# Sukikui/PTI-LDM-VAE

Measured on AMD Instinct MI355X. Metric: vae_train_images_per_sec_256x256, higher is better.
Workload: dtype fp16 forward operands + activations / bf16 backward operands + gradients, fp32 accumulate; 1 GPU; config/vae_dente_no_adv.json 256x256x1 batch 32/GPU: fwd + L1 + 1e-3*KL + bwd + all-reduce + Adam (perceptual term omitted: --perceptual times it; adversarial branch inactive before epoch 6, --adv times it); global_batch=32, parallelism=dp1

## Files before the change

### pti_ldm_vae_amd/csrc/wgrad_mfma.hip

```cpp
#include "pti_common.h"

namespace {

constexpr int TH = 8, TW = 16;
constexpr int PTI_WGRAD_SLAB_V4 = 1 << 30;
#ifndef PTI_WGRAD_BATCH_MAX
#define PTI_WGRAD_BATCH_MAX 16
#endif

struct WgArgs {
  const bf16* x;
  const bf16* dy;
  const stat_t* in_stats;
  const float* gamma;
  const float* beta;
  float* slab;
  int N, H, W, Cin, Ho, Wo, Cout;
  int mode, prologue, groups;
  float eps, inv_cnt;
  int tiles_x, tiles_y, ntiles, S;
  int ci_tiles;
  long long slab_stride;
  int x_f16;
  int diag;
// ... 983 lines not shown
  const int jb = gword & 15, split = gword >> 4, cc = pos - b.grp_start[xcd][gi];
  const W4Job& a = b.job[jb];
  const int ci_pairs = a.Cin / (32 * C::NCH);
  typedef short v4s __attribute__((ext_vector_type(4)));
  typedef short v8s __attribute__((ext_vector_type(8)));
  __shared__ __attribute__((aligned(16))) unsigned char smem[C::LDS];
  const unsigned lds0 = (unsigned)(size_t)(__attribute__((address_space(3))) unsigned char*)smem;
  const int tid = threadIdx.x, lane = tid & 63;
  const int w8 = __builtin_amdgcn_readfirstlane(tid >> 6);
  const int cb = w8 % C::NCB, ch = (w8 / C::NCB) % C::NCH, rg = w8 / (C::NCB * C::NCH);
  const int cotb = cc / ci_pairs, citb = cc % ci_pairs;
  const int co0 = cotb * 32 * C::NCB, ci0 = citb * 32 * C::NCH;
  const bool do_bias = (citb == 0) && (ch == 0);

  int H = a.H, W = a.W;
  asm volatile("" : "+s"(H), "+s"(W));
  int ldsoff[C::NSLOT];
  int yy[C::NSLOT], xx[C::NSLOT], rel[C::NSLOT];
  bool pv[C::NSLOT];
  {
    const int pix = lane >> 2, piece = lane & 3;
#pragma unroll
    for (int k = 0; k < C::KX; ++k) {
      const int xi = w8 + 8 * k;
      const bool sink = xi >= C::NX;
      const int h = xi / C::XI, i = xi - C::XI * h, p = 16 * i + pix;
      ldsoff[k] = sink ? C::STG : h * C::XSUB + i * 1024;
      pv[k] = !sink && p < C::NPX;
      yy[k] = p / HWp - 1;
      xx[k] = p - (p / HWp) * HWp - 1;
      rel[k] = (yy[k] * W + xx[k]) * a.Cin * 2 + (ci0 + h * 32 + piece * 8) * 2;
    }
#pragma unroll
    for (int k = C::KX; k < C::NSLOT; ++k) {
      const int di = w8 + 8 * (k - C::KX), c = di / C::TH_, i = di % C::TH_;
      ldsoff[k] = C::XB + c * C::DSUB + i * 1024;
      pv[k] = true;
      yy[k] = i;
      xx[k] = pix;
      rel[k] = (i * W + pix) * a.Cout * 2 + (co0 + c * 32 + piece * 8) * 2;
    }
#pragma unroll
    for (int k = 0; k < C::NSLOT; ++k) ldsoff[k] = __builtin_amdgcn_readfirstlane(ldsoff[k]);
  }
  const unsigned char* xb = reinterpret_cast<const unsigned char*>(a.x);
  const unsigned char* db = reinterpret_cast<const unsigned char*>(a.dy);
  const unsigned char* zero = reinterpret_cast<const unsigned char*>(pti_wgrad_zero_page);
  struct TilePos { const unsigned char* xt; const unsigned char* dt; int oy0, ox0; };
  auto locate = [&](int tile) -> TilePos {
    TilePos tp;
    const bool live = tile < a.ntiles;
    int t = live ? tile : 0;
    const int tx_ = t % a.tiles_x; t /= a.tiles_x;
    const int ty_ = t % a.tiles_y;
    const int n = t / a.tiles_y;
    tp.oy0 = live ? ty_ * C::TH_ : 1 << 24; tp.ox0 = tx_ * TW;
    const size_t pix0 = (size_t)(n * H + ty_ * C::TH_) * W + tp.ox0;
    tp.xt = xb + pix0 * a.Cin * 2;
    tp.dt = db + pix0 * a.Cout * 2;
    return tp;
  };
  auto issue_slot = [&](const TilePos& tp, int stage, int k) {
    if (b.diag & 1) return;
    const unsigned sb = __builtin_amdgcn_readfirstlane(lds0 + stage * C::STGS + ldsoff[k]);
    const bool ok = pv[k] && (unsigned)(tp.oy0 + yy[k]) < (unsigned)H && (unsigned)(tp.ox0 + xx[k]) < (unsigned)W;
    glds16(ok ? (k < C::KX ? tp.xt : tp.dt) + rel[k] : zero, sb);
  };

  f32x16 acc[3][3];
  float bsum = 0.f;
#pragma unroll
  for (int r = 0; r < 16; ++r)
#pragma unroll
    for (int kh = 0; kh < 3; ++kh)
#pragma unroll
      for (int kw = 0; kw < 3; ++kw) acc[kh][kw][r] = 0.f;
  const int g = lane >> 4, q = (lane & 15) >> 2, pp = lane & 3;
  const int fbase = (8 * (g >> 1) + q) * PP + (16 * (g & 1) + 4 * pp) * 2;
  auto tr_frag = [&](const unsigned char* p) -> bf16x8 {
    const v4s d0 = __builtin_amdgcn_ds_read_tr16_b64_v4i16((v4s __attribute__((address_space(3)))*)(p));
    const v4s d1 = __builtin_amdgcn_ds_read_tr16_b64_v4i16((v4s __attribute__((address_space(3)))*)(p + 4 * PP));
    const v8s t = {d0[0], d0[1], d0[2], d0[3], d1[0], d1[1], d1[2], d1[3]};
    return __builtin_bit_cast(bf16x8, t);
  };

  const int ntl = a.ntiles > split ? (a.ntiles - split + a.S - 1) / a.S : 0;
  auto tile_of = [&](int k) { return k < ntl ? split + k * a.S : a.ntiles; };
#pragma unroll
  for (int s = 0; s < C::DP; ++s) {
    const TilePos tp = locate(tile_of(s));
#pragma unroll
    for (int k = 0; k < C::NSLOT; ++k) issue_slot(tp, s, k);
  }
  bf16x8 dfr[4], xcur, xq1;
  auto xfrag_at = [&](const unsigned char* lX, int f) { return tr_frag(lX + fbase + ((4 * rg + f / 3) * HWp + f % 3) * PP); };
  auto dfrag_at = [&](const unsigned char* lS, int r) { return tr_frag(lS + C::XB + cb * C::DSUB + fbase + (4 * rg + r) * TW * PP); };
  wait_vmcnt<C::NSLOT * (C::DP - 1)>();
  __builtin_amdgcn_s_barrier();
#pragma unroll
  for (int r = 0; r < 4; ++r) dfr[r] = dfrag_at(smem, r);
  xcur = xfrag_at(smem + ch * C::XSUB, 0);
  xq1 = xfrag_at(smem + ch * C::XSUB, 1);

  int ps = 0;
  for (int it = 0; it < ntl; ++it) {
    int fs = ps + C::DP;
    fs = fs >= C::NST ? fs - C::NST : fs;
    const int ns = ps + 1 == C::NST ? 0 : ps + 1;
    const TilePos ft = locate(tile_of(it + C::DP));
    wait_vmcnt<C::NSLOT * (C::DP - 2)>();
    __builtin_amdgcn_s_barrier();
    const unsigned char* lX = smem + ps * C::STGS + ch * C::XSUB;
    const unsigned char* lN = smem + ns * C::STGS;
    if (b.diag & 2) {
#pragma unroll
      for (int k = 0; k < C::NSLOT; ++k) issue_slot(ft, fs, k);
      ps = ns;
      continue;
    }
    if (do_bias) {
#pragma unroll
      for (int r = 0; r < 4; ++r) {
        const u32x4 dwv = __builtin_bit_cast(u32x4, dfr[r]);
        float s8 = 0.f;
#pragma unroll
        for (int i = 0; i < 4; ++i) s8 += __uint_as_float(dwv[i] << 16) + __uint_as_float(dwv[i] & 0xffff0000u);
        bsum += s8;
      }
    }
    bf16x8 dnx[4];
#pragma unroll
    for (int f = 0; f < 18; ++f) {
      const int rr = f / 3, kw = f % 3;
      bf16x8 xq2 = f + 2 < 18 ? xfrag_at(lX, f + 2) : xfrag_at(lN + ch * C::XSUB, f + 2 - 18);
      if (kw == 0 && rr >= 2) dnx[rr - 2] = dfrag_at(lN, rr - 2);
#pragma unroll
      for (int kh = 0; kh < 3; ++kh) {
        const int r = rr - kh;
        if (r >= 0 && r < 4) acc[kh][kw] = __builtin_amdgcn_mfma_f32_32x32x16_bf16(dfr[r], xcur, acc[kh][kw], 0, 0, 0);
      }
      if (C::NSLOT == 4) {
        if (f == 2) issue_slot(ft, fs, 0);
        if (f == 6) issue_slot(ft, fs, 1);
        if (f == 10) issue_slot(ft, fs, 2);
        if (f == 14) issue_slot(ft, fs, 3);
      } else {
        if (f == 2) issue_slot(ft, fs, 0);
        if (f == 5) issue_slot(ft, fs, 1);
        if (f == 8) issue_slot(ft, fs, 2);
        if (f == 11) issue_slot(ft, fs, 3);
        if (f == 14) issue_slot(ft, fs, C::NSLOT - 1);
      }
      if (kw == 0 && rr >= 2) __builtin_amdgcn_sched_group_barrier(0x100, 4, 0);
      else __builtin_amdgcn_sched_group_barrier(0x100, 2, 0);
      {
        const int nm = (rr == 0 || rr == 5) ? 1 : ((rr == 1 || rr == 4) ? 2 : 3);
        if (nm == 3) __builtin_amdgcn_sched_group_barrier(0x008, 3, 0);
        else if (nm == 2) __builtin_amdgcn_sched_group_barrier(0x008, 2, 0);
        else __builtin_amdgcn_sched_group_barrier(0x008, 1, 0);
      }
      __builtin_amdgcn_sched_barrier(0);
      xcur = xq1;
      xq1 = xq2;
    }
#pragma unroll
    for (int r = 0; r < 4; ++r) dfr[r] = dnx[r];
    ps = ns;
  }
  wait_vmcnt<0>();

  const int ci = lane & 31, hsel = lane >> 5;
  if (do_bias) bsum += __shfl_xor(bsum, 32, 64);
  if constexpr (C::NRG == 2) {
    __syncthreads();
    float* red = reinterpret_cast<float*>(smem) + (cb + C::NCB * ch) * 5120;
    float* bred = reinterpret_cast<float*>(smem) + C::NCB * C::NCH * 5120;
#pragma unroll
    for (int round = 0; round < 2; ++round) {
      if (round) __syncthreads();
      if (rg == 1) {
#pragma unroll
        for (int t = 0; t < 9; ++t)
          if ((t < 5) == (round == 0))
#pragma unroll
            for (int q4 = 0; q4 < 4; ++q4)
              *(f32x4*)(red + (t - 5 * round) * 1024 + ci * 32 + (((2 * q4 + hsel) ^ (ci & 7)) << 2)) =
                  f32x4{acc[t / 3][t % 3][4 * q4], acc[t / 3][t % 3][4 * q4 + 1], acc[t / 3][t % 3][4 * q4 + 2], acc[t / 3][t % 3][4 * q4 + 3]};
        if (round == 0 && do_bias && lane < 32) bred[cb * 32 + lane] = bsum;
      }
      __syncthreads();
      if (rg == 0) {
#pragma unroll
        for (int t = 0; t < 9; ++t)
          if ((t < 5) == (round == 0))
#pragma unroll
            for (int q4 = 0; q4 < 4; ++q4) {
              const f32x4 v = *(const f32x4*)(red + (t - 5 * round) * 1024 + ci * 32 + (((2 * q4 + hsel) ^ (ci & 7)) << 2));
#pragma unroll
              for (int j = 0; j < 4; ++j) acc[t / 3][t % 3][4 * q4 + j] += v[j];
            }
        if (round == 0 && do_bias && lane < 32) bsum += bred[cb * 32 + lane];
      }
    }
    if (rg == 1) return;
  }
  const int cc32 = (C::NCB * cotb + cb) * (a.Cin / 32) + C::NCH * citb + ch;
  float* blk = a.slab + (size_t)split * a.slab_stride + (size_t)cc32 * 9216;
#pragma unroll
  for (int kh = 0; kh < 3; ++kh)
#pragma unroll
    for (int kw = 0; kw < 3; ++kw)
#pragma unroll
      for (int q4 = 0; q4 < 4; ++q4)
        *(f32x4*)(blk + (kh * 3 + kw) * 1024 + ci * 32 + (((2 * q4 + hsel) ^ (ci & 7)) << 2)) =
            f32x4{acc[kh][kw][4 * q4], acc[kh][kw][4 * q4 + 1], acc[kh][kw][4 * q4 + 2], acc[kh][kw][4 * q4 + 3]};
  if (do_bias && lane < 32) a.slab[(size_t)split * a.slab_stride + (size_t)9 * a.Cout * a.Cin + co0 + cb * 32 + lane] = bsum;
}

__global__ __launch_bounds__(256) void wgrad_reduce4_kernel(W4Batch b) {
  __shared__ f32x4 red[16][16];
  int jb = 0;
  while (jb + 1 < b.njobs && (int)blockIdx.x >= b.first_rblk[jb + 1]) ++jb;
  const W4Job& a = b.job[jb];
  const float* __restrict__ slab = a.slab;
  float* __restrict__ dw = b.dw[jb];
  float* __restrict__ dbias = b.dbias[jb];
  const int S = a.S, Cout = a.Cout, Cin = a.Cin, accumulate = b.accumulate[jb];
  const long long stride = a.slab_stride;
  const long long total = (long long)9 * Cout * Cin;
  const int col = threadIdx.x & 15, sg = threadIdx.x >> 4;
  const long long e = ((long long)(blockIdx.x - b.first_rblk[jb]) * 16 + col) * 4;
  f32x4 s0 = {0.f, 0.f, 0.f, 0.f}, s1 = s0;
  if (e < total + Cout) {
    int k = sg;
    for (; k + 16 < S; k += 32) {
      s0 += *(const f32x4*)(slab + (size_t)k * stride + e);
      s1 += *(const f32x4*)(slab + (size_t)(k + 16) * stride + e);
    }
    if (k < S) s0 += *(const f32x4*)(slab + (size_t)k * stride + e);
  }
  red[sg][col] = s0 + s1;
  __syncthreads();
  if (sg == 0 && e < total + Cout) {
    f32x4 sum = red[0][col];
#pragma unroll
    for (int g = 1; g < 16; ++g) sum += red[g][col];
    if (e < total) {
      const int cc = (int)(e / 9216), i = (int)(e % 9216);
      const int ci_tiles = Cin / 32;
      const int co0 = (cc / ci_tiles) * 32, ci0 = (cc % ci_tiles) * 32;
      const int tap = i >> 10, ci = (i >> 5) & 31, cog = ((i >> 2) & 7) ^ (ci & 7);
#pragma unroll
      for (int j = 0; j < 4; ++j) {
        const size_t o = ((size_t)(co0 + cog * 4 + j) * Cin + ci0 + ci) * 9 + tap;
        dw[o] = accumulate ? dw[o] + sum[j] : sum[j];
      }
    } else if (dbias) {
      const int co = (int)(e - total);
#pragma unroll
      for (int j = 0; j < 4; ++j) dbias[co + j] = accumulate ? dbias[co + j] + sum[j] : sum[j];
    }
  }
}

__global__ __launch_bounds__(256) void wgrad_reduce_kernel(const float* __restrict__ slab, long long stride, int S,
                                                           float* __restrict__ dw, float* __restrict__ dbias, int Cout,
                                                           int Cin, int KK, int accumulate) {
  __shared__ f32x4 red[16][16];
  const long long total = (long long)KK * Cout * Cin;
  const int col = threadIdx.x & 15, sg = threadIdx.x >> 4;
  const long long e = ((long long)blockIdx.x * 16 + col) * 4;
  f32x4 s0 = {0.f, 0.f, 0.f, 0.f}, s1 = s0;
  if (e < total + Cout) {
    int k = sg;
    for (; k + 16 < S; k += 32) {
      s0 += *(const f32x4*)(slab + (size_t)k * stride + e);
      s1 += *(const f32x4*)(slab + (size_t)(k + 16) * stride + e);
    }
    if (k < S) s0 += *(const f32x4*)(slab + (size_t)k * stride + e);
  }
  red[sg][col] = s0 + s1;
  __syncthreads();
  if (sg == 0 && e < total + Cout) {
    f32x4 sum = red[0][col];
#pragma unroll
    for (int g = 1; g < 16; ++g) sum += red[g][col];
    if (e < total) {
      const int ci = e % Cin;
      const int co = (e / Cin) % Cout;
      const int t = e / ((long long)Cin * Cout);
#pragma unroll
      for (int j = 0; j < 4; ++j) {
        const size_t o = ((size_t)co * Cin + ci + j) * KK + t;
        dw[o] = accumulate ? dw[o] + sum[j] : sum[j];
      }
    } else if (dbias) {
      const int co = (int)(e - total);
#pragma unroll
      for (int j = 0; j < 4; ++j) dbias[co + j] = accumulate ? dbias[co + j] + sum[j] : sum[j];
    }
  }
}

template <int KS, int S_, int CO_T, int CI_T>
void launch_w(const WgArgs& a, int grid_y, hipStream_t st) {
  if (a.prologue == PTI_PRO_NONE)
    PTI_LAUNCH((wgrad_mfma_kernel<KS, S_, CO_T, CI_T, true>), dim3(grid_y, a.S), dim3(256), 0, st, a);
  else
    PTI_LAUNCH((wgrad_mfma_kernel<KS, S_, CO_T, CI_T, false>), dim3(grid_y, a.S), dim3(256), 0, st, a);
}
template <int KS, int S_>
void launch_wt(const WgArgs& a, int co_t, int ci_t, int grid_y, hipStream_t st) {
  if (co_t == 64 && ci_t == 64) launch_w<KS, S_, 64, 64>(a, grid_y, st);
  else if (co_t == 64) launch_w<KS, S_, 64, 32>(a, grid_y, st);
  else if (ci_t == 64) launch_w<KS, S_, 32, 64>(a, grid_y, st);
  else launch_w<KS, S_, 32, 32>(a, grid_y, st);
}

}

static int w6_mode(int n, int h, int w, int cin, int cout) {
  const char* e = getenv("PTI_WGRAD_V6");
  const int v = e ? atoi(e) : 3;
  if (v >= 1 && cout % 128 == 0 && cin % 64 == 0) return 2;
  if (v >= 2 && cout % 64 == 0 && cin % 64 == 0 && (v == 2 || (long long)h * w <= 128 * 128)) return 3;
  return 0;
}
static void w4_fill_job(W4Job& a, const void* x, const void* dy, int n, int h, int w, int cin, int cout, int mode) {
  a.x = (const bf16*)x; a.dy = (const bf16*)dy; a.slab = nullptr;
  a.N = n; a.H = h; a.W = w; a.Cin = cin; a.Cout = cout;
  a.tiles_x = cdiv(w, TW); a.tiles_y = cdiv(h, mode == 2 ? W6A::TH_ : TH); a.ntiles = n * a.tiles_x * a.tiles_y;
  a.slab_stride = (long long)9 * cout * cin + cout;
  a.S = 1;
  a.cob2 = mode;
}
static bool w4_eligible(int n, int h, int w, int cin, int cout) {
  return n > 0 && h > 0 && w > 0 && cin > 0 && cout > 0 && cin % 32 == 0 && cout % 32 == 0 &&
         (long long)n * h * w * cin * 2 < (1ll << 31) && (long long)n * h * w * cout * 2 < (1ll << 31);
}
static int w4_mode(int cout) {
  static const int cob2_env = getenv("PTI_WGRAD_V4_COB2") ? atoi(getenv("PTI_WGRAD_V4_COB2")) : 1;
  return (cob2_env && cout % 64 == 0) ? 1 : 0;
}
extern "C" int pti_conv_wgrad_batched_mode(int n, int h, int w, int cin, int cout) {
  if (!w4_eligible(n, h, w, cin, cout)) return PTI_EUNSUPPORTED;
  const int v4 = w4_mode(cout), v6 = w6_mode(n, h, w, cin, cout);
  return v6 ? v6 : v4;
}
static int wgrad_diag_env() {
  const char* v = getenv("PTI_WGRAD_V4_DIAG");
  const char* ok = getenv("PTI_ALLOW_WRONG_RESULTS");
  if (!v || atoi(v) == 0) return 0;
  if (!ok || atoi(ok) != 1) {
    fprintf(stderr, "[pti] PTI_WGRAD_V4_DIAG ignored: it needs PTI_ALLOW_WRONG_RESULTS=1 (results are garbage)\n");
    return 0;
  }
  fprintf(stderr, "[pti] WRONG-RESULT DIAGNOSTIC ACTIVE: PTI_WGRAD_V4_DIAG=%s\n", v);
  return atoi(v);
}
static long long w4_plan(W4Batch& b, float* workspace, long long workspace_floats) {
  static const int wgs_env = getenv("PTI_WGRAD_V4_WGS") ? atoi(getenv("PTI_WGRAD_V4_WGS")) : 2048;
  static const int diag_env = wgrad_diag_env();
  b.diag = diag_env;
  auto tiles32 = [](const W4Job& a) {
    return a.cob2 == 2 ? (a.Cin / 64) * (a.Cout / 128) : a.cob2 == 3 ? (a.Cin / 64) * (a.Cout / 64)
                                                                     : (a.Cin / 32) * (a.Cout / (a.cob2 ? 64 : 32));
  };
  const bool m6 = b.njobs > 0 && b.job[0].cob2 >= 2;
  const char* w6e = getenv("PTI_WGRAD_V6_WGS");
  const int wgs6 = w6e && atoi(w6e) > 0 ? atoi(w6e) : 512;
  double work = 0;
  for (int j = 0; j < b.njobs; ++j) work += (double)tiles32(b.job[j]) * (b.job[j].cob2 == 1 ? 2 : 1) * b.job[j].ntiles;
  double per_wg = work / wgs_env > 2.0 ? work / wgs_env : 2.0;
  if (m6) per_wg = work / wgs6 > 4.0 ? work / wgs6 : 4.0;
  for (int attempt = 0;; ++attempt) {
    long long used = 0;
    int rb = 0, groups = 0;
    bool fits = true;
    for (int j = 0; j < b.njobs; ++j) {
      W4Job& a = b.job[j];
      int S = (int)((double)a.ntiles * (a.cob2 == 1 ? 2 : 1) / per_wg + 0.5);
      if (S > a.ntiles / (a.cob2 ? 1 : 2)) S = a.ntiles / (a.cob2 ? 1 : 2);
      if (S > 255) S = 255;
      if (S < 1) S = 1;
      if (used + (long long)S * a.slab_stride > workspace_floats) fits = false;
      a.S = S;
      a.slab = workspace + used;
      used += (long long)S * a.slab_stride;
      groups += S;
      b.first_rblk[j] = rb;
      rb += (int)((a.slab_stride / 4 + 15) / 16);
    }
    b.first_rblk[b.njobs] = rb;
    if (fits && groups <= 8 * W4_MAXGRP) {
      int len[8] = {0, 0, 0, 0, 0, 0, 0, 0};
      for (int x = 0; x < 8; ++x) { b.ngrp[x] = 0; b.grp_start[x][0] = 0; }
      int order[PTI_WGRAD_BATCH_MAX];
      for (int j = 0; j < b.njobs; ++j) order[j] = j;
      for (int i = 0; i < b.njobs; ++i)
        for (int j = i + 1; j < b.njobs; ++j)
          if (tiles32(b.job[order[j]]) > tiles32(b.job[order[i]])) { const int t = order[i]; order[i] = order[j]; order[j] = t; }
      bool ok = true;
      for (int i = 0; i < b.njobs && ok; ++i) {
        const int j = order[i];
        for (int sp = 0; sp < b.job[j].S; ++sp) {
          int best = 0;
          for (int x = 1; x < 8; ++x)
            if (len[x] < len[best]) best = x;
          if (b.ngrp[best] >= W4_MAXGRP || len[best] + tiles32(b.job[j]) > 65535) { ok = false; break; }
          b.grp[best][b.ngrp[best]] = (unsigned short)((unsigned)j | ((unsigned)sp << 4));
          len[best] += tiles32(b.job[j]);
          b.grp_start[best][++b.ngrp[best]] = (unsigned short)len[best];
        }
      }
      if (ok) {
        int mx = 0;
        for (int x = 0; x < 8; ++x) mx = len[x] > mx ? len[x] : mx;
        b.nwg = 8 * mx;
        return used;
      }
    }
    if (attempt > 40) return -1;
    per_wg *= 1.25;
  }
}

extern "C" int64_t pti_conv_wgrad_workspace_bytes(int cout, int cin, int ksize, int splits) {
  return (int64_t)splits * ((int64_t)ksize * ksize * cout * cin + cout) * 4;
}

static int wgrad_check(const void* x, const void* dy, const int64_t* in_stats, const float* gamma, const float* beta,
                       const void* workspace, const pti_conv_desc* d) {
  if (!x || !dy || !workspace || !d) PTI_FAIL(PTI_EINVAL, "conv_wgrad_mfma: null pointer");
  if (d->cin % 32 || d->cout % 32) PTI_FAIL(PTI_EUNSUPPORTED, "conv_wgrad_mfma: cin=%d cout=%d", d->cin, d->cout);
  if (d->ksize != 1 && d->ksize != 3) PTI_FAIL(PTI_EUNSUPPORTED, "conv_wgrad_mfma: ksize");
  if (d->mode == PTI_CONV_ZINS || (d->ksize == 1 && d->mode != PTI_CONV_S1)) PTI_FAIL(PTI_EUNSUPPORTED, "conv_wgrad_mfma: mode %d", d->mode);
  if (d->prologue != PTI_PRO_NONE && (!in_stats || !gamma || !beta || d->groups <= 0 || d->cin % d->groups))
    PTI_FAIL(PTI_EINVAL, "conv_wgrad_mfma: prologue args");
  return PTI_OK;
}

extern "C" int pti_conv_wgrad_mfma_partials(const void* x, const void* dy, const int64_t* in_stats, const float* gamma,
                                            const float* beta, void* workspace, int64_t workspace_bytes,
                                            const pti_conv_desc* d, int* splits_out, pti_stream_t s) {
  if (!splits_out) PTI_FAIL(PTI_EINVAL, "conv_wgrad_mfma_partials: null splits_out");
  if (int rc = wgrad_check(x, dy, in_stats, gamma, beta, workspace, d)) return rc;
  WgArgs a;
  a.x = (const bf16*)x; a.dy = (const bf16*)dy; a.in_stats = (const stat_t*)in_stats; a.gamma = gamma; a.beta = beta;
  a.slab = (float*)workspace;
  a.N = d->n; a.H = d->h; a.W = d->w; a.Cin = d->cin; a.Ho = d->ho; a.Wo = d->wo; a.Cout = d->cout;
  a.mode = d->mode; a.prologue = d->prologue; a.groups = d->groups; a.eps = d->eps; a.x_f16 = d->in_f16;
  static const int diag_env = wgrad_diag_env();
  a.diag = diag_env;
  a.inv_cnt = d->prologue != PTI_PRO_NONE ? 1.0f / ((float)(d->cin / d->groups) * (float)d->h * (float)d->w) : 0.f;
  a.tiles_x = cdiv(d->wo, TW); a.tiles_y = cdiv(d->ho, TH); a.ntiles = d->n * a.tiles_x * a.tiles_y;
  int co_t = d->cout % 64 == 0 ? 64 : 32, ci_t = d->cin % 64 == 0 ? 64 : 32;
  if ((long long)a.ntiles * (d->cout / co_t) * (d->cin / ci_t) < 16 * 512) co_t = ci_t = 32;
  const bool v3 = d->ksize == 3 && d->mode != PTI_CONV_S2PAD;
  static const int cob_env = getenv("PTI_WGRAD_COB") ? atoi(getenv("PTI_WGRAD_COB")) : 0;
  const bool cob_ok = d->cout % 64 == 0 && d->mode == PTI_CONV_S1;
  const int cob = (cob_ok && cob_env != 1 && (cob_env == 2 || d->prologue != PTI_PRO_NONE)) ? 2 : 1;
  if (v3) { ci_t = 32; co_t = 32 * cob; }
  a.ci_tiles = d->cin / ci_t;
  const int tiles_cc = (d->cout / co_t) * a.ci_tiles;
  const int kk = d->ksize * d->ksize;
  a.slab_stride = (long long)kk * d->cout * d->cin + d->cout;
  const long long smax = workspace_bytes / (a.slab_stride * 4);
  const bool plain = d->prologue == PTI_PRO_NONE && cob == 1;
  static const int v1_wgs = getenv("PTI_WGRAD_V1_WGS") ? atoi(getenv("PTI_WGRAD_V1_WGS")) : 512;
  int S = (v3 ? (cob == 2 ? 512 : (plain ? (tiles_cc == 1 ? 1024 : 1280) : 768)) : v1_wgs) / tiles_cc;
  if (S > a.ntiles / 4) S = a.ntiles / 4;
  const int scap = v3 ? (plain ? 1024 : 512) : 256;
  if (S > scap) S = scap;
  if (S < 1) S = 1;
  if (S > smax) S = (int)smax;
  if (S < 1) PTI_FAIL(PTI_EINVAL, "conv_wgrad_mfma: workspace too small (%lld bytes per split needed)", a.slab_stride * 4);
  static const int v4_env = getenv("PTI_WGRAD_V4") ? atoi(getenv("PTI_WGRAD_V4")) : 1;
  const bool v4 = v3 && v4_env && d->prologue == PTI_PRO_NONE && !d->in_f16 && d->mode == PTI_CONV_S1 &&
                  w4_eligible(d->n, d->h, d->w, d->cin, d->cout);
  if (v4) {
    W4Batch b;
    b.njobs = 1;
    w4_fill_job(b.job[0], x, dy, d->n, d->h, d->w, d->cin, d->cout, pti_conv_wgrad_batched_mode(d->n, d->h, d->w, d->cin, d->cout));
    b.dw[0] = b.dbias[0] = nullptr;
    b.accumulate[0] = 0;
    if (w4_plan(b, (float*)workspace, workspace_bytes / 4) < 0)
      PTI_FAIL(PTI_EINVAL, "conv_wgrad_mfma: workspace too small (%lld bytes per split needed)", a.slab_stride * 4);
    const char* v5e = getenv("PTI_WGRAD_V5");
    const bool v5 = v5e && atoi(v5e) != 0 && !b.diag;
    if (b.job[0].cob2 == 2) PTI_LAUNCH(wgrad_mfma6_kernel<W6A>, dim3(b.nwg), dim3(512), 0, (hipStream_t)s, b);
    else if (b.job[0].cob2 == 3) PTI_LAUNCH(wgrad_mfma6_kernel<W6B>, dim3(b.nwg), dim3(512), 0, (hipStream_t)s, b);
    else if (b.job[0].cob2 && v5) PTI_LAUNCH(wgrad_mfma5_kernel, dim3(b.nwg), dim3(256), 0, (hipStream_t)s, b);
    else if (b.job[0].cob2) PTI_LAUNCH(wgrad_mfma4_kernel<true>, dim3(b.nwg), dim3(512), 0, (hipStream_t)s, b);
    else PTI_LAUNCH(wgrad_mfma4_kernel<false>, dim3(b.nwg), dim3(512), 0, (hipStream_t)s, b);
    PTI_CHECK_LAUNCH("conv_wgrad_mfma");
    *splits_out = b.job[0].S | PTI_WGRAD_SLAB_V4;
    return PTI_OK;
  }
  if (v3 && S >= 8) S &= ~7;
  a.S = S;
  hipStream_t st = (hipStream_t)s;
  if (v3 && cob == 2) PTI_LAUNCH((wgrad_mfma3_kernel<2, false>), dim3(tiles_cc * S), dim3(192), 0, st, a);
  else if (v3 && plain) PTI_LAUNCH((wgrad_mfma3_kernel<1, true>), dim3(tiles_cc * S), dim3(192), 0, st, a);
  else if (v3) PTI_LAUNCH((wgrad_mfma3_kernel<1, false>), dim3(tiles_cc * S), dim3(192), 0, st, a);
  else if (d->ksize == 1) launch_wt<1, 1>(a, co_t, ci_t, tiles_cc, st);
  else launch_wt<3, 2>(a, co_t, ci_t, tiles_cc, st);
  PTI_CHECK_LAUNCH("conv_wgrad_mfma");
  *splits_out = S;
  return PTI_OK;
}

extern "C" int pti_conv_wgrad_reduce(const void* workspace, int splits, float* dw, float* dbias, int accumulate,
                                     const pti_conv_desc* d, pti_stream_t s) {
  if (!workspace || !dw || !d || splits < 1) PTI_FAIL(PTI_EINVAL, "conv_wgrad_reduce: bad arguments");
  const int kk = d->ksize * d->ksize;
  const long long total = (long long)kk * d->cout * d->cin + d->cout;
  if (splits & PTI_WGRAD_SLAB_V4) {
    if (kk != 9 || !w4_eligible(d->n, d->h, d->w, d->cin, d->cout)) PTI_FAIL(PTI_EINVAL, "conv_wgrad_reduce: block-ordered slabs are 3x3 only");
    W4Batch b;
    b.njobs = 1;
    w4_fill_job(b.job[0], nullptr, nullptr, d->n, d->h, d->w, d->cin, d->cout, w4_mode(d->cout));
    b.job[0].S = splits & ~PTI_WGRAD_SLAB_V4;
    b.job[0].slab = (float*)workspace;
    b.dw[0] = dw; b.dbias[0] = dbias; b.accumulate[0] = accumulate;
    b.diag = 0; b.nwg = 0;
    for (int x = 0; x < 8; ++x) b.ngrp[x] = 0;
    b.first_rblk[0] = 0;
    b.first_rblk[1] = (int)((total / 4 + 15) / 16);
    PTI_LAUNCH(wgrad_reduce4_kernel, dim3(b.first_rblk[1]), dim3(256), 0, (hipStream_t)s, b);
    PTI_CHECK_LAUNCH("conv_wgrad_reduce");
    return PTI_OK;
  }
  PTI_LAUNCH(wgrad_reduce_kernel, dim3((unsigned)((total / 4 + 15) / 16)), dim3(256), 0, (hipStream_t)s,
                     (const float*)workspace, total, splits, dw, dbias, d->cout, d->cin, kk, accumulate);
  PTI_CHECK_LAUNCH("conv_wgrad_reduce");
  return PTI_OK;
}

extern "C" int pti_conv_wgrad_mfma(const void* x, const void* dy, const int64_t* in_stats, const float* gamma,
                                   const float* beta, float* dw, float* dbias, void* workspace,
                                   int64_t workspace_bytes, int accumulate, const pti_conv_desc* d, pti_stream_t s) {
  if (!dw) PTI_FAIL(PTI_EINVAL, "conv_wgrad_mfma: null pointer");
  int splits = 0;
  if (int rc = pti_conv_wgrad_mfma_partials(x, dy, in_stats, gamma, beta, workspace, workspace_bytes, d, &splits, s)) return rc;
  return pti_conv_wgrad_reduce(workspace, splits, dw, dbias, accumulate, d, s);
}

extern "C" int pti_conv_wgrad_mfma_batched(const pti_wgrad_job* jobs, int njobs, void* workspace, int64_t workspace_bytes,
                                           pti_stream_t s) {
  if (!jobs || !workspace || njobs < 1 || njobs > PTI_WGRAD_BATCH_MAX)
    PTI_FAIL(PTI_EINVAL, "conv_wgrad_mfma_batched: 1..%d jobs", PTI_WGRAD_BATCH_MAX);
  W4Batch bm[4];
  bm[0].njobs = bm[1].njobs = bm[2].njobs = bm[3].njobs = 0;
  for (int j = 0; j < njobs; ++j) {
    const pti_wgrad_job& q = jobs[j];
    if (!q.x || !q.dy || !q.dw) PTI_FAIL(PTI_EINVAL, "conv_wgrad_mfma_batched: job %d has a null pointer", j);
    const int mode = pti_conv_wgrad_batched_mode(q.n, q.h, q.w, q.cin, q.cout);
    if (mode < 0)
      PTI_FAIL(PTI_EUNSUPPORTED, "conv_wgrad_mfma_batched: job %d: n=%d h=%d w=%d cin=%d cout=%d (channels must be multiples of 32, tensors < 2 GiB)",
               j, q.n, q.h, q.w, q.cin, q.cout);
    W4Job jb;
    w4_fill_job(jb, q.x, q.dy, q.n, q.h, q.w, q.cin, q.cout, mode);
    W4Batch& b = bm[mode];
    const int k = b.njobs++;
    b.job[k] = jb;
    b.dw[k] = q.dw; b.dbias[k] = q.dbias; b.accumulate[k] = q.accumulate;
  }
  float* ws = (float*)workspace;
  long long ws_floats = workspace_bytes / 4;
  const char* v5e = getenv("PTI_WGRAD_V5");
  const int v5_env = v5e ? atoi(v5e) : 0;
  const void* main_kernel = nullptr;
  long long need[4] = {0, 0, 0, 0}, need_all = 0;
  for (int m = 0; m < 4; ++m) {
    for (int j = 0; j < bm[m].njobs; ++j) need[m] += bm[m].job[j].slab_stride;
    need_all += need[m];
  }
  if (need_all > ws_floats) PTI_FAIL(PTI_EINVAL, "conv_wgrad_mfma_batched: workspace too small (%lld bytes needed for one split per job)", need_all * 4);
  const long long ws_total = ws_floats;
  for (int m = 3; m >= 0; --m) {
    W4Batch& b = bm[m];
    if (b.njobs == 0) continue;
    long long later = 0;
    for (int m2 = m - 1; m2 >= 0; --m2) later += need[m2];
    long long avail = (long long)((double)ws_total * ((double)need[m] / (double)need_all));
    if (avail < need[m]) avail = need[m];
    if (later == 0 || avail > ws_floats - later) avail = ws_floats - later;
    const long long used = w4_plan(b, ws, avail);
    if (used < 0) PTI_FAIL(PTI_EINVAL, "conv_wgrad_mfma_batched: workspace too small");
    ws += used;
    ws_floats -= used;
    const void* kfn;
    if (m == 3) { PTI_LAUNCH(wgrad_mfma6_kernel<W6B>, dim3(b.nwg), dim3(512), 0, (hipStream_t)s, b); kfn = reinterpret_cast<const void*>(wgrad_mfma6_kernel<W6B>); }
    else if (m == 2) { PTI_LAUNCH(wgrad_mfma6_kernel<W6A>, dim3(b.nwg), dim3(512), 0, (hipStream_t)s, b); kfn = reinterpret_cast<const void*>(wgrad_mfma6_kernel<W6A>); }
    else if (m == 1 && v5_env && !b.diag) { PTI_LAUNCH(wgrad_mfma5_kernel, dim3(b.nwg), dim3(256), 0, (hipStream_t)s, b); kfn = reinterpret_cast<const void*>(wgrad_mfma5_kernel); }
    else if (m == 1) { PTI_LAUNCH(wgrad_mfma4_kernel<true>, dim3(b.nwg), dim3(512), 0, (hipStream_t)s, b); kfn = reinterpret_cast<const void*>(wgrad_mfma4_kernel<true>); }
    else { PTI_LAUNCH(wgrad_mfma4_kernel<false>, dim3(b.nwg), dim3(512), 0, (hipStream_t)s, b); kfn = reinterpret_cast<const void*>(wgrad_mfma4_kernel<false>); }
    PTI_CHECK_LAUNCH("conv_wgrad_mfma_batched");
    if (!main_kernel) main_kernel = kfn;
    PTI_LAUNCH(wgrad_reduce4_kernel, dim3(b.first_rblk[b.njobs]), dim3(256), 0, (hipStream_t)s, b);
    PTI_CHECK_LAUNCH("conv_wgrad_mfma_batched reduce");
  }
  pti_last_kernel = main_kernel;
  return PTI_OK;
}
```

Before: 2710 images/s.

## Add dedicated 1x1 conv weight-gradient MFMA kernel with pixel-staged double buffering

Adds a specialised wgrad kernel for 1x1 convolutions that treats the problem as a plain GEMM over flattened pixels. It stages x and dy channel tiles through double-buffered, swizzled LDS, reads them with transposing LDS loads into 32x32x16 bf16 MFMAs, and fuses the GroupNorm/SiLU prologue and the bias reduction. Split-K is sized from stage count and byte volume. This replaces the generic spatial-tile path for ksize==1, which wasted work on halo and tile logic. The cost is added code complexity, and the swizzle and transpose-load indexing carry correctness risk.

```diff
diff --git a/pti_ldm_vae_amd/csrc/wgrad_mfma.hip b/pti_ldm_vae_amd/csrc/wgrad_mfma.hip
--- a/pti_ldm_vae_amd/csrc/wgrad_mfma.hip
+++ b/pti_ldm_vae_amd/csrc/wgrad_mfma.hip
@@ -1309,6 +1309,260 @@
   }
 }
 
+struct K1Args {
+  const bf16* x; const bf16* dy; const stat_t* in_stats; const float* gamma; const float* beta; float* slab;
+  long long slab_stride;
+  int P, HW, Cin, Cout, prologue, groups, nstages, S, ci_tiles, x_f16;
+  float eps, inv_cnt;
+};
+
+template <int CO_B, int CI_B>
+struct K1Cfg {
+  static constexpr int SUM = CO_B + CI_B;
+  static constexpr int SP = SUM >= 192 ? 64 : (SUM >= 96 ? 128 : 256);
+  static constexpr int MB = CO_B / 32, NB = CI_B / 32;
+  static constexpr int WCO = MB >= 2 ? 2 : 1, WCI = NB >= 2 ? 2 : 1, WPX = 4 / (WCO * WCI);
+  static constexpr int MI = MB / WCO, NI = NB / WCI;
+  static constexpr int RA = CI_B * 2, RD = CO_B * 2;
+  static constexpr int NCA = CI_B / 8, NCD = CO_B / 8;
+  static constexpr int A_BYTES = SP * RA, D_BYTES = SP * RD, STG = A_BYTES + D_BYTES;
+  static constexpr int AIT = SP * NCA / 256, DIT = SP * NCD / 256;
+  static constexpr int KBW = SP / 16 / WPX;
+  static constexpr int RED_BYTES = (WPX - 1) * WCO * WCI * MI * NI * 4096;
+  static constexpr int BIAS_BYTES = 8 * 256 * 4;
+  static constexpr int LDS0 = 2 * STG > RED_BYTES ? 2 * STG : RED_BYTES;
+  static constexpr int LDS_BYTES = LDS0 > BIAS_BYTES ? LDS0 : BIAS_BYTES;
+  static_assert(SP * NCA % 256 == 0 && SP * NCD % 256 == 0 && (SP / 16) % WPX == 0, "stage must divide over the threads");
+};
+template <int CB> __device__ __forceinline__ int k1_swz(int pixel) {
+  return CB == 128 ? (pixel & 3) << 6 : (CB == 64 ? ((pixel >> 1) & 1) << 6 : 0);
+}
+
+template <int CO_B, int CI_B, bool PLAIN>
+__global__ __launch_bounds__(256, 2) void wgrad_k1_kernel(K1Args a) {
+  using C = K1Cfg<CO_B, CI_B>;
+  typedef short v4s __attribute__((ext_vector_type(4)));
+  typedef short v8s __attribute__((ext_vector_type(8)));
+  __shared__ __attribute__((aligned(16))) unsigned char smem[C::LDS_BYTES];
+  const int prologue = PLAIN ? PTI_PRO_NONE : a.prologue;
+  const bool x_f16 = PLAIN ? false : (bool)a.x_f16;
+  const int tid = threadIdx.x, lane = tid & 63, wave = tid >> 6;
+  const int split = blockIdx.y;
+  const int cot = blockIdx.x / a.ci_tiles, cit = blockIdx.x % a.ci_tiles;
+  const int wco = wave / (C::WCI * C::WPX), wci = (wave / C::WPX) % C::WCI, wpx = wave % C::WPX;
+  const int sb = (int)((long long)a.nstages * split / a.S), se = (int)((long long)a.nstages * (split + 1) / a.S);
+  const int nst = se - sb;
+
+  const int g = lane >> 4, q = (lane & 15) >> 2, pp = lane & 3;
+  const int pk = 8 * (g >> 1) + q, chl = 16 * (g & 1) + 4 * pp;
+  int dl[C::MI], al[C::NI];
+#pragma unroll
+  for (int mi = 0; mi < C::MI; ++mi) dl[mi] = pk * C::RD + ((((wco * C::MI + mi) * 32 + chl) * 2) ^ k1_swz<CO_B>(q));
+#pragma unroll
+  for (int ni = 0; ni < C::NI; ++ni) al[ni] = pk * C::RA + ((((wci * C::NI + ni) * 32 + chl) * 2) ^ k1_swz<CI_B>(q));
+
+  f32x16 acc[C::MI][C::NI];
+#pragma unroll
+  for (int mi = 0; mi < C::MI; ++mi)
+#pragma unroll
+    for (int ni = 0; ni < C::NI; ++ni)
+#pragma unroll
+      for (int r = 0; r < 16; ++r) acc[mi][ni][r] = 0.f;
+  float bsum[8];
+#pragma unroll
+  for (int j = 0; j < 8; ++j) bsum[j] = 0.f;
+
+  const int alc = tid % C::NCA, alp = tid / C::NCA;
+  const int dlc = tid % C::NCD, dlp = tid / C::NCD;
+  constexpr int APSTEP = 256 / C::NCA, DPSTEP = 256 / C::NCD;
+  const int awr = alp * C::RA + ((alc * 16) ^ k1_swz<CI_B>(alp));
+  const int dwr = dlp * C::RD + ((dlc * 16) ^ k1_swz<CO_B>(dlp));
+  const bf16* xg = a.x + (size_t)alp * a.Cin + cit * CI_B + alc * 8;
+  const bf16* dg = a.dy + (size_t)dlp * a.Cout + cot * CO_B + dlc * 8;
+  const bool do_bias = (cit == 0);
+  const int cpg = a.Cin / (a.groups > 0 ? a.groups : 1);
+  int cur_n = -1;
+  float sc[8], sh[8];
+
+  auto issue = [&](u32x4 (&ra)[C::AIT], u32x4 (&rd)[C::DIT], int stage) {
+    const int p0 = stage * C::SP;
+#pragma unroll
+    for (int it = 0; it < C::AIT; ++it) {
+      const int p = p0 + alp + it * APSTEP;
+      ra[it] = u32x4{0u, 0u, 0u, 0u};
+      if (p < a.P) ra[it] = *(const u32x4*)(xg + (size_t)(p0 + it * APSTEP) * a.Cin);
+    }
+#pragma unroll
+    for (int it = 0; it < C::DIT; ++it) {
+      const int p = p0 + dlp + it * DPSTEP;
+      rd[it] = u32x4{0u, 0u, 0u, 0u};
+      if (p < a.P) rd[it] = *(const u32x4*)(dg + (size_t)(p0 + it * DPSTEP) * a.Cout);
+    }
+  };
+  auto set_sample = [&](int stage) {
+    if (PLAIN || prologue == PTI_PRO_NONE) return;
+    const int n = (stage * C::SP) / a.HW;
+    if (n == cur_n) return;
+    cur_n = n;
+#pragma unroll
+    for (int j = 0; j < 8; ++j) {
+      const int ch = cit * CI_B + alc * 8 + j;
+      const int gg = ch / cpg;
+      const float sum = stat_f(a.in_stats, (n * a.groups + gg) * 2), sq = stat_f(a.in_stats, (n * a.groups + gg) * 2 + 1);
+      const float mean = sum * a.inv_cnt;
+      const float rstd = rsqrtf(fmaxf(sq * a.inv_cnt - mean * mean, 0.f) + a.eps);
+      sc[j] = rstd * a.gamma[ch];
+      sh[j] = a.beta[ch] - mean * sc[j];
+    }
+  };
+  auto commit = [&](u32x4 (&ra)[C::AIT], u32x4 (&rd)[C::DIT], int stage, int slot) {
+    unsigned char* lA = smem + slot * C::STG;
+    unsigned char* lD = lA + C::A_BYTES;
+    set_sample(stage);
+#pragma unroll
+    for (int it = 0; it < C::AIT; ++it) {
+      u32x4 r = ra[it];
+      if (!PLAIN) {
+        if (prologue != PTI_PRO_NONE) {
+          float f[8];
+          unpack8f(r, f, x_f16);
+#pragma unroll
+          for (int j = 0; j < 8; ++j) {
+            float v = f[j] * sc[j] + sh[j];
+            if (prologue == PTI_PRO_GN_SILU) v = silu_f(v);
+            f[j] = v;
+          }
+          r = pack8(f);
+        } else if (x_f16) {
+          float f[8];
+          unpack8f(r, f, true);
+          r = pack8(f);
+        }
+      }
+      *(u32x4*)(lA + awr + it * APSTEP * C::RA) = r;
+    }
+#pragma unroll
+    for (int it = 0; it < C::DIT; ++it) {
+      *(u32x4*)(lD + dwr + it * DPSTEP * C::RD) = rd[it];
+      if (do_bias) {
+        float f[8];
+        unpack8(rd[it], f);
+#pragma unroll
+        for (int j = 0; j < 8; ++j) bsum[j] += f[j];
+      }
+    }
+  };
+  auto compute = [&](int slot) {
+    const unsigned char* lA = smem + slot * C::STG;
+    const unsigned char* lD = lA + C::A_BYTES;
+#pragma unroll
+    for (int kk = 0; kk < C::KBW; ++kk) {
+      const int kb = wpx + kk * C::WPX;
+      bf16x8 dfr[C::MI], afr[C::NI];
+#pragma unroll
+      for (int mi = 0; mi < C::MI; ++mi) {
+        const unsigned char* p = lD + kb * 16 * C::RD + dl[mi];
+        const v4s r0 = __builtin_amdgcn_ds_read_tr16_b64_v4i16((v4s __attribute__((address_space(3)))*)(p));
+        const v4s r1 = __builtin_amdgcn_ds_read_tr16_b64_v4i16((v4s __attribute__((address_space(3)))*)(p + 4 * C::RD));
+        const v8s t8 = {r0[0], r0[1], r0[2], r0[3], r1[0], r1[1], r1[2], r1[3]};
+        dfr[mi] = __builtin_bit_cast(bf16x8, t8);
+      }
+#pragma unroll
+      for (int ni = 0; ni < C::NI; ++ni) {
+        const unsigned char* p = lA + kb * 16 * C::RA + al[ni];
+        const v4s r0 = __builtin_amdgcn_ds_read_tr16_b64_v4i16((v4s __attribute__((address_space(3)))*)(p));
+        const v4s r1 = __builtin_amdgcn_ds_read_tr16_b64_v4i16((v4s __attribute__((address_space(3)))*)(p + 4 * C::RA));
+        const v8s t8 = {r0[0], r0[1], r0[2], r0[3], r1[0], r1[1], r1[2], r1[3]};
+        afr[ni] = __builtin_bit_cast(bf16x8, t8);
+      }
+#pragma unroll
+      for (int mi = 0; mi < C::MI; ++mi)
+#pragma unroll
+        for (int ni = 0; ni < C::NI; ++ni)
+          acc[mi][ni] = __builtin_amdgcn_mfma_f32_32x32x16_bf16(dfr[mi], afr[ni], acc[mi][ni], 0, 0, 0);
+    }
+  };
+
+  u32x4 ra0[C::AIT], rd0[C::DIT], ra1[C::AIT], rd1[C::DIT];
+  if (nst > 0) set_sample(sb);
+  if (nst > 0) issue(ra0, rd0, sb);
+  if (nst > 1) issue(ra1, rd1, sb + 1);
+  if (nst > 0) commit(ra0, rd0, sb, 0);
+  if (nst > 2) issue(ra0, rd0, sb + 2);
+  __syncthreads();
+  for (int j = 0; j < nst; j += 2) {
+    compute(0);
+    if (j + 1 < nst) commit(ra1, rd1, sb + j + 1, 1);
+    if (j + 3 < nst) issue(ra1, rd1, sb + j + 3);
+    __syncthreads();
+    if (j + 1 < nst) {
+      compute(1);
+      if (j + 2 < nst) commit(ra0, rd0, sb + j + 2, 0);
+      if (j + 4 < nst) issue(ra0, rd0, sb + j + 4);
+      __syncthreads();
+    }
+  }
+
+  float* slab = a.slab + (size_t)split * a.slab_stride;
+  float* red = reinterpret_cast<float*>(smem);
+  const int hsel = lane >> 5;
+#pragma unroll
+  for (int mi = 0; mi < C::MI; ++mi)
+#pragma unroll
+    for (int ni = 0; ni < C::NI; ++ni) {
+      if constexpr (C::WPX > 1) {
+        if (wpx > 0) {
+          float* dst = red + ((wco * C::WCI + wci) * (C::WPX - 1) + (wpx - 1)) * 1024;
+#pragma unroll
+          for (int r = 0; r < 16; ++r) dst[r * 64 + lane] = acc[mi][ni][r];
+        }
+        __syncthreads();
+        if (wpx == 0) {
+#pragma unroll
+          for (int o = 0; o < C::WPX - 1; ++o) {
+            const float* src = red + ((wco * C::WCI + wci) * (C::WPX - 1) + o) * 1024;
+#pragma unroll
+            for (int r = 0; r < 16; ++r) acc[mi][ni][r] += src[r * 64 + lane];
+          }
+        }
+        __syncthreads();
+      }
+      if (wpx == 0) {
+        const int ci = cit * CI_B + (wci * C::NI + ni) * 32 + (lane & 31);
+#pragma unroll
+        for (int r = 0; r < 16; ++r) {
+          const int co = cot * CO_B + (wco * C::MI + mi) * 32 + (r & 3) + 8 * (r >> 2) + 4 * hsel;
+          slab[(size_t)co * a.Cin + ci] = acc[mi][ni][r];
+        }
+      }
+    }
+  if (do_bias) {
+#pragma unroll
+    for (int j = 0; j < 8; ++j) red[j * 256 + tid] = bsum[j];
+    __syncthreads();
+    if (tid < CO_B) {
+      const int lc = tid / 8, j = tid % 8;
+      float s = 0.f;
+      for (int k = lc; k < 256; k += C::NCD) s += red[j * 256 + k];
+      slab[(size_t)a.Cout * a.Cin + cot * CO_B + tid] = s;
+    }
+  }
+}
+
+template <int CO_B, int CI_B>
+void launch_k1b(const K1Args& a, bool plain, dim3 grid, hipStream_t st) {
+  if (plain) PTI_LAUNCH((wgrad_k1_kernel<CO_B, CI_B, true>), grid, dim3(256), 0, st, a);
+  else PTI_LAUNCH((wgrad_k1_kernel<CO_B, CI_B, false>), grid, dim3(256), 0, st, a);
+}
+template <int CO_B>
+void launch_k1a(const K1Args& a, int ci_b, bool plain, dim3 grid, hipStream_t st) {
+  if (ci_b == 128) launch_k1b<CO_B, 128>(a, plain, grid, st);
+  else if (ci_b == 64) launch_k1b<CO_B, 64>(a, plain, grid, st);
+  else launch_k1b<CO_B, 32>(a, plain, grid, st);
+}
+static int k1_block(int c) { return c % 128 == 0 ? 128 : (c % 64 == 0 ? 64 : 32); }
+static int k1_stage_pixels(int co_b, int ci_b) { return co_b + ci_b >= 192 ? 64 : (co_b + ci_b >= 96 ? 128 : 256); }
+
 template <int KS, int S_, int CO_T, int CI_T>
 void launch_w(const WgArgs& a, int grid_y, hipStream_t st) {
   if (a.prologue == PTI_PRO_NONE)
@@ -1447,6 +1701,42 @@
   return PTI_OK;
 }
 
+static bool k1_launch(const WgArgs& w, const pti_conv_desc* d, int64_t workspace_bytes, int* splits_out, hipStream_t st) {
+  const char* e = getenv("PTI_WGRAD_K1");
+  if (e && atoi(e) == 0) return false;
+  const long long P = (long long)d->n * d->h * d->w;
+  if (P < 1 || P >= (1ll << 31) || d->ho != d->h || d->wo != d->w) return false;
+  const int co_b = k1_block(d->cout), ci_b = k1_block(d->cin), sp = k1_stage_pixels(co_b, ci_b);
+  if (d->prologue != PTI_PRO_NONE && ((long long)d->h * d->w) % sp != 0) return false;
+  K1Args a;
+  a.x = w.x; a.dy = w.dy; a.in_stats = w.in_stats; a.gamma = w.gamma; a.beta = w.beta; a.slab = w.slab;
+  a.slab_stride = (long long)d->cout * d->cin + d->cout;
+  a.P = (int)P; a.HW = d->h * d->w; a.Cin = d->cin; a.Cout = d->cout; a.prologue = d->prologue; a.groups = d->groups;
+  a.x_f16 = d->in_f16; a.eps = d->eps; a.inv_cnt = w.inv_cnt;
+  a.nstages = (int)((P + sp - 1) / sp);
+  a.ci_tiles = d->cin / ci_b;
+  const int tiles_cc = (d->cout / co_b) * a.ci_tiles;
+  const long long smax = workspace_bytes / (a.slab_stride * 4);
+  if (smax < 1) return false;
+  const char* we = getenv("PTI_WGRAD_K1_WGS");
+  const int wgs = we && atoi(we) > 0 ? atoi(we) : 512;
+  long long S = wgs / tiles_cc;
+  if (S > a.nstages / 4) S = a.nstages / 4;
+  const long long by_bytes = P * (d->cin + d->cout) * 2 / (2 * a.slab_stride * 4);
+  if (S > by_bytes) S = by_bytes;
+  if (S > 65535) S = 65535;
+  if (S > smax) S = smax;
+  if (S < 1) S = 1;
+  a.S = (int)S;
+  const bool plain = d->prologue == PTI_PRO_NONE && !d->in_f16;
+  const dim3 grid(tiles_cc, a.S);
+  if (co_b == 128) launch_k1a<128>(a, ci_b, plain, grid, st);
+  else if (co_b == 64) launch_k1a<64>(a, ci_b, plain, grid, st);
+  else launch_k1a<32>(a, ci_b, plain, grid, st);
+  *splits_out = a.S;
+  return true;
+}
+
 extern "C" int pti_conv_wgrad_mfma_partials(const void* x, const void* dy, const int64_t* in_stats, const float* gamma,
                                             const float* beta, void* workspace, int64_t workspace_bytes,
                                             const pti_conv_desc* d, int* splits_out, pti_stream_t s) {
@@ -1461,6 +1751,10 @@
   a.diag = diag_env;
   a.inv_cnt = d->prologue != PTI_PRO_NONE ? 1.0f / ((float)(d->cin / d->groups) * (float)d->h * (float)d->w) : 0.f;
   a.tiles_x = cdiv(d->wo, TW); a.tiles_y = cdiv(d->ho, TH); a.ntiles = d->n * a.tiles_x * a.tiles_y;
+  if (d->ksize == 1 && k1_launch(a, d, workspace_bytes, splits_out, (hipStream_t)s)) {
+    PTI_CHECK_LAUNCH("conv_wgrad_mfma (k1)");
+    return PTI_OK;
+  }
   int co_t = d->cout % 64 == 0 ? 64 : 32, ci_t = d->cin % 64 == 0 ? 64 : 32;
   if ((long long)a.ntiles * (d->cout / co_t) * (d->cin / ci_t) < 16 * 512) co_t = ci_t = 32;
   const bool v3 = d->ksize == 3 && d->mode != PTI_CONV_S2PAD;
```

Result: no change. 2727 images/s, median of 6 (+0.7%).
